# speechcatcher-asr/speechcatcher

Measured on AMD Instinct MI355X. Metric: concurrent real-time streams (audio-seconds/s), de_xl dims, 640 ms (10240-sample) chunk steps, beam 10 CTC+attention, higher is better.
Workload: dtype f32

## Files before the change

speechcatcher_amd/csrc/search.hip:

```cpp
#include "common.h"
#include "attn.h"
#include <mutex>
#include <unordered_map>

#define CTRL(s, f) sb.ctrl[(s) * 8 + (f)]
#define SC_CTC_T(s) (CTRL(s, SC_C_TCTC) > 0 ? CTRL(s, SC_C_TCTC) : CTRL(s, SC_C_T))

#define YSEQ(pp, s, h) (sb.yseq + (((long)(pp) * sb.S + (s)) * sb.W + (h)) * sb.LCAP)
#define XPOS(pp, s, h) (sb.xpos + (((long)(pp) * sb.S + (s)) * sb.W + (h)) * sb.LCAP)
#define ANC(pp, s) (sb.anc + ((long)(pp) * sb.S + (s)) * sb.LCAP * sb.W)
#define CTCR(pp, s) (sb.ctc_r + ((long)(pp) * sb.S + (s)) * sb.TCAP * 2 * sb.W)
#define CTCRS(pp, s) (sb.ctc_rs + ((long)(pp) * sb.S + (s)) * sb.TCAP * sb.W)

__global__ void ctc_extend_state_kernel(sc_search sb) {
  const int s = blockIdx.x, h = threadIdx.x;
  if (!CTRL(s, SC_C_ACTIVE) || !CTRL(s, SC_C_HAS)) return;
  const int T = CTRL(s, SC_C_T), told = CTRL(s, SC_C_TOLD), nh = CTRL(s, SC_C_NHYP);
  if (h >= nh || told >= T) return;
  float *r = CTCR(CTRL(s, SC_C_CUR), s);
  float *rs = CTCRS(CTRL(s, SC_C_CUR), s);
  const float *x = sb.ctcx + (long)s * sb.TCAP * sb.V;
  const int t0 = told < 1 ? 1 : told;
  float rb = r[((long)(t0 - 1) * 2 + 1) * sb.W + h];
  for (int t = t0; t < T; ++t) {
    rb = rb + x[(long)t * sb.V + sb.blank];
    r[((long)t * 2 + 0) * sb.W + h] = SC_LOGZERO;
    r[((long)t * 2 + 1) * sb.W + h] = rb;
    rs[(long)t * sb.W + h] = rb;
  }
}

__global__ __launch_bounds__(256) void ctc_table_transpose_kernel(sc_search sb) {
  __shared__ float tile[32][33];
  const int s = blockIdx.z;
  if (!CTRL(s, SC_C_ACTIVE)) return;
  const int T = CTRL(s, SC_C_T), told = CTRL(s, SC_C_TOLD);
  if (told >= T) return;
  const int V = sb.V, v0 = blockIdx.x * 32;
  const int tx = threadIdx.x & 31, ty = threadIdx.x >> 5;
  const float *x = sb.ctcx + (long)s * sb.TCAP * V;
  float *xt = sb.ctcxT + (long)s * V * sb.tct;
  for (int t0 = (told & ~31) + blockIdx.y * 32; t0 < T; t0 += gridDim.y * 32) {
#pragma unroll
    for (int j = 0; j < 4; ++j) {
      const int t = t0 + ty + 8 * j, v = v0 + tx;
      tile[ty + 8 * j][tx] = (t < T && v < V) ? x[(long)t * V + v] : 0.f;
    }
    __syncthreads();
#pragma unroll
    for (int j = 0; j < 4; ++j) {
      const int v = v0 + ty + 8 * j, t = t0 + tx;
      if (v < V && t >= told && t < T) xt[(long)v * sb.tct + t] = tile[tx][ty + 8 * j];
    }
    __syncthreads();
  }
}

extern "C" int sc_ctc_extend_state(const sc_search *sbp, void *stream) {
  SC_CHECK_ARG(sbp, "null");
  if (sbp->ctcxT)
    ctc_table_transpose_kernel<<<dim3(cdiv(sbp->V, 32), 4, sbp->S), 256, 0, (hipStream_t)stream>>>(*sbp);
  ctc_extend_state_kernel<<<sbp->S, 64, 0, (hipStream_t)stream>>>(*sbp);
  SC_CHECK_LAUNCH();
  return SC_OK;
}

__global__ void kv_rows_to_half_kernel(const float *stage, const int32_t *rows, int m, int TCAP, int d2, _Float16 *ckv) {
  const int li = blockIdx.y;
  for (long e = (long)blockIdx.x * blockDim.x + threadIdx.x; e < (long)m * d2; e += (long)gridDim.x * blockDim.x) {
    const int j = (int)(e / d2), c = (int)(e % d2);
    ckv[((long)rows[j] + (long)li * TCAP) * d2 + c] = (_Float16)stage[((long)li * m + j) * d2 + c];
  }
}

extern "C" int sc_kv_rows_to_half(const float *stage, const int32_t *rows, int m, int n_layers, int TCAP, int d2,
                                  void *ckv_half, void *stream) {
  SC_CHECK_ARG(stage && rows && ckv_half && m >= 0 && n_layers > 0 && d2 > 0, "bad arguments");
  if (m == 0) return SC_OK;
  const int gx = (int)(((long)m * d2 + 255) / 256 > 1024 ? 1024 : ((long)m * d2 + 255) / 256);
  kv_rows_to_half_kernel<<<dim3(gx, n_layers), 256, 0, (hipStream_t)stream>>>(stage, rows, m, TCAP, d2, (_Float16 *)ckv_half);
  SC_CHECK_LAUNCH();
  return SC_OK;
}

#define SC_KV_MAX_ROWS 65536
__global__ void dec_embed_kernel(sc_search sb, float sq) {
  const int row = blockIdx.x, s = row / sb.W, h = row % sb.W;
  if (!CTRL(s, SC_C_ACTIVE) || h >= CTRL(s, SC_C_NHYP)) return;
  const int L = CTRL(s, SC_C_L);
  const int tok = YSEQ(CTRL(s, SC_C_CUR), s, h)[L - 1];
  for (int c = threadIdx.x; c < sb.d; c += blockDim.x)
    sb.dx[(long)row * sb.d + c] = sb.embed[(long)tok * sb.d + c] * sq + sb.pe[(long)(L - 1) * sb.d + c];
}

extern "C" int sc_dec_embed(const sc_search *sbp, void *stream) {
  SC_CHECK_ARG(sbp, "null");
  dec_embed_kernel<<<sbp->S * sbp->W, 256, 0, (hipStream_t)stream>>>(*sbp, sqrtf((float)sbp->d));
  SC_CHECK_LAUNCH();
  return SC_OK;
}

template <int DK, int WM, bool SELF, int UNR, bool KVH = false>
__global__ __launch_bounds__(256, (UNR <= 4 && WM <= 10 && DK <= 32) ? 4 : 1) void dec_attn_flash_kernel(sc_search sb, int li) {
  constexpr int PCH = 128;
  constexpr int NTW = (UNR >= 8) ? 4 : 2;
  constexpr int NP = SELF ? 5 : 4;
  extern __shared__ __attribute__((aligned(16))) float smem[];
  const int head = blockIdx.x, s = sb.rowmap ? sb.rowmap[blockIdx.y * sb.W] / sb.W : blockIdx.y;
  if (!CTRL(s, SC_C_ACTIVE)) return;
  const int nh = CTRL(s, SC_C_NHYP);
  if (nh <= 0) return;
  const int L = CTRL(s, SC_C_L), cur = CTRL(s, SC_C_CUR), T = CTRL(s, SC_C_T);
  const int W = sb.W, d = sb.d;
  const int tid = threadIdx.x, lane = tid & 63, wave = tid >> 6;
  float *pm = smem;
  float *pl = pm + NP * 16;
  float *pO = pl + NP * 16;
  int *rows = (int *)(smem + mattn_partial_floats(DK, NP));
  int *wtot = rows + (SELF ? PCH * W : 0);
  float *qs = (float *)(wtot + 8);

  const float *qbase = SELF ? sb.dqkv + (long)s * W * 3 * d + head * DK : sb.dq + (long)s * W * d + head * DK;
  const int qld = SELF ? 3 * d : d;
  const long skv0 = ((long)s * sb.n_layers + li) * sb.kv_rows * 2 * d + head * DK;
  const long ckv0 = ((long)s * sb.n_layers + li) * sb.TCAP * 2 * d + head * DK;
  if (SELF) {
    const int *ancn = ANC(cur, s) + (long)(L - 1) * W;
    for (int e = tid; e < nh * DK; e += 256) {
      const int h = e / DK, c = e % DK;
      const long dst = skv0 + (long)ancn[h] * 2 * d;
      kv_store1<KVH>(sb.skv, dst + c, qbase[(long)h * 3 * d + d + c]);
      kv_store1<KVH>(sb.skv, dst + d + c, qbase[(long)h * 3 * d + 2 * d + c]);
    }
  }
  const float scale = sqrtf((float)DK);
  for (int e = tid; e < 16 * DK; e += 256) {
    const int h = e / DK, c = e % DK;
    qs[e] = h < nh ? qbase[(long)h * qld + c] / scale : 0.f;
  }
  MAttn<DK> st;
  mattn_init(st);

  if (SELF) {
    const int *anc = ANC(cur, s);
    const int Lc = L - 1;
    const int nchunk = cdiv(Lc, PCH);
    if (nchunk == 0) __syncthreads();
    int urows = nh;
    for (int ch = 0; ch < nchunk; ++ch) {
      const int c0 = ch * PCH;
      const int nopre[WM] = {};
      const int U = mattn_build_rows<WM>(rows, wtot, anc, c0, Lc, W, nh, tid, lane, wave, nopre);
      urows += U;
      mattn_walk<DK, NTW, KVH>(st, qs, sb.skv, d, cdiv(U, 16), wave, lane, [&](int idx, long &ke, unsigned &hm) {
        const int e = rows[min(idx, max(U - 1, 0))];
        hm = idx < U ? (unsigned)e >> 16 : 0u;
// ... 204 lines not shown

__device__ __forceinline__ int next_pow2(int v) {
  int n = 1;
  while (n < v) n <<= 1;
  return n;
}

__device__ __forceinline__ unsigned long long shfl_xor_u64(unsigned long long v, int mask) {
  const unsigned lo = __shfl_xor((unsigned)v, mask, 64), hi = __shfl_xor((unsigned)(v >> 32), mask, 64);
  return ((unsigned long long)hi << 32) | lo;
}
__device__ __forceinline__ unsigned long long shfl_u64(unsigned long long v, int src) {
  const unsigned lo = __shfl((unsigned)v, src, 64), hi = __shfl((unsigned)(v >> 32), src, 64);
  return ((unsigned long long)hi << 32) | lo;
}
__device__ __forceinline__ unsigned long long wave_sort64_desc(unsigned long long v, int lane) {
#pragma unroll
  for (int k = 2; k <= 64; k <<= 1) {
#pragma unroll
    for (int j = k >> 1; j > 0; j >>= 1) {
      const unsigned long long o = shfl_xor_u64(v, j);
      const bool keep_max = ((lane & j) == 0) == ((lane & k) == 0);
      v = keep_max ? (v > o ? v : o) : (v < o ? v : o);
    }
  }
  return v;
}
__device__ __forceinline__ unsigned long long wave_merge64_desc(unsigned long long a, unsigned long long b, int lane) {
  const unsigned long long br = shfl_u64(b, 63 - lane);
  unsigned long long v = a > br ? a : br;
#pragma unroll
  for (int j = 32; j > 0; j >>= 1) {
    const unsigned long long o = shfl_xor_u64(v, j);
    v = ((lane & j) == 0) ? (v > o ? v : o) : (v < o ? v : o);
  }
  return v;
}

__global__ __launch_bounds__(256) void logsoftmax_topk_kernel(sc_search sb) {
  __shared__ float red[8];
  __shared__ unsigned long long tops[4][64];
  const int row = blockIdx.x, s = row / sb.W, h = row % sb.W;
  if (!CTRL(s, SC_C_ACTIVE) || h >= CTRL(s, SC_C_NHYP)) return;
  const int V = sb.V, tid = threadIdx.x, lane = tid & 63, wave = tid >> 6;
  const float *x = sb.logits + (long)row * V;
  float xv[4];
  float m = -INFINITY;
#pragma unroll
  for (int q = 0; q < 4; ++q) {
    const int c = wave * 256 + q * 64 + lane;
    xv[q] = c < V ? x[c] : -INFINITY;
    m = fmaxf(m, xv[q]);
  }
  m = wave_max(m);
  if (lane == 0) red[wave] = m;
  __syncthreads();
  m = fmaxf(fmaxf(red[0], red[1]), fmaxf(red[2], red[3]));
  float sum = 0.f;
#pragma unroll
  for (int q = 0; q < 4; ++q) sum += (wave * 256 + q * 64 + lane < V) ? expf(xv[q] - m) : 0.f;
  sum = wave_sum(sum);
  if (lane == 0) red[4 + wave] = sum;
  __syncthreads();
  sum = (red[4] + red[5]) + (red[6] + red[7]);
  const float ls = logf(sum);
  unsigned long long key[4];
#pragma unroll
  for (int q = 0; q < 4; ++q) {
    const int c = wave * 256 + q * 64 + lane;
    if (c < V) {
      const float lp = (xv[q] - m) - ls;
      sb.logp[(long)row * V + c] = lp;
      key[q] = sort_key(__fmul_rn(sb.w_dec, lp), c);
    } else {
      key[q] = 0ull;
    }
  }
#pragma unroll
  for (int q = 0; q < 4; ++q) key[q] = wave_sort64_desc(key[q], lane);
  const unsigned long long m0 = wave_merge64_desc(key[0], key[1], lane);
  const unsigned long long m1 = wave_merge64_desc(key[2], key[3], lane);
  tops[wave][lane] = wave_merge64_desc(m0, m1, lane);
  __syncthreads();
  if (wave == 0) {
    const unsigned long long a = wave_merge64_desc(tops[0][lane], tops[1][lane], lane);
    const unsigned long long b = wave_merge64_desc(tops[2][lane], tops[3][lane], lane);
    const unsigned long long f = wave_merge64_desc(a, b, lane);
    if (lane < sb.K) sb.pre_ids[(long)row * sb.K + lane] = sort_key_index(f);
  }
}

__global__ __launch_bounds__(256) void logsoftmax_topk_sort_kernel(sc_search sb) {
  extern __shared__ __attribute__((aligned(16))) unsigned long long comp[];
  __shared__ float red[8];
  const int row = blockIdx.x, s = row / sb.W, h = row % sb.W;
  if (!CTRL(s, SC_C_ACTIVE) || h >= CTRL(s, SC_C_NHYP)) return;
  const int V = sb.V, tid = threadIdx.x, lane = tid & 63, wave = tid >> 6;
  const int NP = next_pow2(V);
  const float *x = sb.logits + (long)row * V;
  float m = -INFINITY;
  for (int c = tid; c < V; c += 256) m = fmaxf(m, x[c]);
  m = wave_max(m);
  if (lane == 0) red[wave] = m;
  __syncthreads();
  m = fmaxf(fmaxf(red[0], red[1]), fmaxf(red[2], red[3]));
  float sum = 0.f;
  for (int c = tid; c < V; c += 256) sum += expf(x[c] - m);
  sum = wave_sum(sum);
  if (lane == 0) red[4 + wave] = sum;
  __syncthreads();
  sum = (red[4] + red[5]) + (red[6] + red[7]);
  const float ls = logf(sum);
  for (int c = tid; c < NP; c += 256) {
    if (c < V) {
      float lp = (x[c] - m) - ls;
      sb.logp[(long)row * V + c] = lp;
      comp[c] = sort_key(__fmul_rn(sb.w_dec, lp), c);
    } else {
      comp[c] = 0ull;
    }
  }
  __syncthreads();
  block_bitonic_sort_desc(comp, NP);
  for (int k = tid; k < sb.K; k += 256) sb.pre_ids[(long)row * sb.K + k] = sort_key_index(comp[k]);
}

static size_t pow2_keys_bytes(int V) {
  size_t np = 1;
  while (np < (size_t)V) np <<= 1;
  return np * sizeof(unsigned long long);
}
static size_t fuse_topw_lds(int V) { return 2 * (size_t)V * sizeof(float) + pow2_keys_bytes(V); }

extern "C" int sc_logsoftmax_topk(const sc_search *sbp, void *stream) {
  SC_CHECK_ARG(sbp, "null");
  SC_CHECK_ARG(sbp->V > 0 && sbp->V <= SC_MAX_VOCAB, "vocabulary larger than SC_MAX_VOCAB (8192)");
  if (sbp->V <= 1024 && sbp->K <= 64)
    logsoftmax_topk_kernel<<<sbp->S * sbp->W, 256, 0, (hipStream_t)stream>>>(*sbp);
  else {
    const size_t lds = pow2_keys_bytes(sbp->V);
    const int rc = allow_large_lds(reinterpret_cast<const void *>(&logsoftmax_topk_sort_kernel), lds,
                                   pow2_keys_bytes(SC_MAX_VOCAB), "sc_logsoftmax_topk");
    if (rc != SC_OK) return rc;
    logsoftmax_topk_sort_kernel<<<sbp->S * sbp->W, 256, lds, (hipStream_t)stream>>>(*sbp);
  }
  SC_CHECK_LAUNCH();
  return SC_OK;
}

struct CtcChunkT {
  float4 xc[4], xb[4];
  float pn[16], pb[16];
};
#define SC_CTC_CK 16
__host__ __device__ static inline int ctc_tck(int TCAP) { return (TCAP + SC_CTC_CK - 1) / SC_CTC_CK; }
__device__ __forceinline__ void ctc_frame(float &r_n, float &r_b, float prs, float pb, bool same, float xc, float xb, float &phi) {
  phi = same ? pb : prs;
  const float nr_n = lse2(r_n, phi) + xc;
  const float nr_b = lse2(r_n, r_b) + xb;
  r_n = nr_n;
  r_b = nr_b;
}
__device__ __forceinline__ void ctc_psi_add(float &pm, float &ps, float v) {
  const float d = v - pm;
  const float e = sc_exp_neg(-fabsf(d));
  ps = d > 0.f ? ps * e + 1.f : ps + e;
  pm = sc_max_raw(pm, v);
}
__device__ __forceinline__ bool ctc_scan_is_split(int T, int L, int split_min) {
  const int out_len = L - 1;
  int start = out_len > 1 ? out_len : 1;
  if (start > T) start = T;
  return split_min > 0 && T - start >= split_min;
}
#define CTC_NSEG 32
static inline int ctc_split_min_ok(int TCAP, int split_min) { return ctc_tck(TCAP) >= CTC_NSEG ? split_min : 0; }

__global__ __launch_bounds__(256) void ctc_prefix_scan_colmajor_kernel(sc_search sb, int split_min) {
  const int s = blockIdx.y;
  if (!CTRL(s, SC_C_ACTIVE)) return;
  const int nh = CTRL(s, SC_C_NHYP), K = sb.K, W = sb.W, V = sb.V;
  const int e = blockIdx.x * 256 + threadIdx.x;
  if (e >= nh * K) return;
  const int h = e / K, k = e % K;
  const int T = SC_CTC_T(s), L = CTRL(s, SC_C_L), cur = CTRL(s, SC_C_CUR);
  if (ctc_scan_is_split(T, L, split_min)) return;
  const bool has = CTRL(s, SC_C_HAS);
  const long row = (long)s * W + h;
  const int c = sb.pre_ids[row * K + k];
  const int last = YSEQ(cur, s, h)[L - 1];
  const bool same = (c == last);
  const int tct = sb.tct;
  const float *__restrict__ xcol = sb.ctcxT + ((long)s * V + c) * tct;
  const float *__restrict__ xblk = sb.ctcxT + ((long)s * V + sb.blank) * tct;
  const float *__restrict__ rp = CTCR(cur, s);
  const float *__restrict__ rsp = CTCRS(cur, s);
  float *rn = sb.ctc_rnew + (long)s * ctc_tck(sb.TCAP) * 2 * (W * K);
  const int WK = W * K;
  const int out_len = L - 1;
  int start = out_len > 1 ? out_len : 1;
  if (start > T) start = T;
  for (int j = 0; SC_CTC_CK * j + SC_CTC_CK - 1 < start - 1; ++j) {
    rn[((long)j * 2) * WK + e] = SC_LOGZERO;
    rn[((long)j * 2 + 1) * WK + e] = SC_LOGZERO;
  }
  float r_n = (out_len == 0) ? xcol[0] : SC_LOGZERO;
  float r_b = SC_LOGZERO;
  if (((start - 1) & (SC_CTC_CK - 1)) == SC_CTC_CK - 1) {
    rn[((long)((start - 1) / SC_CTC_CK) * 2) * WK + e] = r_n;
    rn[((long)((start - 1) / SC_CTC_CK) * 2 + 1) * WK + e] = r_b;
  }
  float cum = 0.f;
  if (!has)
    for (int t = 0; t < start; ++t) cum += xblk[t];

  auto fetch = [&](CtcChunkT &q, int tb) {
#pragma unroll
    for (int j = 0; j < 4; ++j) {
      const int t4 = min(tb + 4 * j, tct - 4);
      q.xc[j] = *reinterpret_cast<const float4 *>(xcol + t4);
      q.xb[j] = *reinterpret_cast<const float4 *>(xblk + t4);
    }
    if (has) {
#pragma unroll
      for (int i = 0; i < 16; ++i) {
        int t = tb + i;
        t = t < T ? (t < 1 ? 1 : t) : T - 1;
        q.pn[i] = rsp[(long)(t - 1) * W + h];
        q.pb[i] = rp[((long)(t - 1) * 2 + 1) * W + h];
      }
    }
  };
  float pm = r_n, ps = 1.f;
  auto frame = [&](const CtcChunkT &q, int tb, int i) {
    const int t = tb + i;
    const float4 c4 = q.xc[i >> 2], b4 = q.xb[i >> 2];
    const float xc = (i & 3) == 0 ? c4.x : (i & 3) == 1 ? c4.y : (i & 3) == 2 ? c4.z : c4.w;
    const float xb = (i & 3) == 0 ? b4.x : (i & 3) == 1 ? b4.y : (i & 3) == 2 ? b4.z : b4.w;
    const float prs = has ? q.pn[i] : cum;
    const float pb = has ? q.pb[i] : cum;
    float phi;
    ctc_frame(r_n, r_b, prs, pb, same, xc, xb, phi);
    if ((i & (SC_CTC_CK - 1)) == SC_CTC_CK - 1) {
      rn[((long)(t / SC_CTC_CK) * 2) * WK + e] = r_n;
      rn[((long)(t / SC_CTC_CK) * 2 + 1) * WK + e] = r_b;
    }
    ctc_psi_add(pm, ps, phi + xc);
    if (!has) cum += xb;
  };
  auto advance = [&](const CtcChunkT &q, int tb) {
    if (tb >= start && tb + 16 <= T) {
#pragma unroll
      for (int i = 0; i < 16; ++i) frame(q, tb, i);
    } else {
#pragma unroll
      for (int i = 0; i < 16; ++i)
        if (tb + i >= start && tb + i < T) frame(q, tb, i);
    }
  };
  if (start < T) {
    CtcChunkT qa, qb;
    int tb = start & ~15;
    fetch(qa, tb);
    while (true) {
      if (tb + 16 < T) fetch(qb, tb + 16);
      advance(qa, tb);
      tb += 16;
      if (tb >= T) break;
      if (tb + 16 < T) fetch(qa, tb + 16);
      advance(qb, tb);
      tb += 16;
      if (tb >= T) break;
    }
  }
  float psi = pm + logf(ps);
  const float rsum_last = has ? rsp[(long)(T - 1) * W + h] : cum;
  if (c == sb.eos) psi = rsum_last;
  if (c == sb.blank) psi = SC_LOGZERO;
  sb.psi[row * K + k] = psi;
  if (k == 0) sb.psi_eos[row] = rsum_last;
}

#define CTC_EB (256 / CTC_NSEG)
__global__ __launch_bounds__(256) void ctc_prefix_scan_tpar_kernel(sc_search sb, int split_min) {
  __shared__ float co[8][CTC_NSEG][CTC_EB];
  __shared__ float st0[2][CTC_NSEG][CTC_EB];
  __shared__ float cum0[CTC_NSEG][CTC_EB];
  const int s = blockIdx.y;
  if (!CTRL(s, SC_C_ACTIVE)) return;
  const int nh = CTRL(s, SC_C_NHYP), K = sb.K, W = sb.W, V = sb.V;
  const int T = SC_CTC_T(s), L = CTRL(s, SC_C_L), cur = CTRL(s, SC_C_CUR);
  if (!ctc_scan_is_split(T, L, split_min)) return;
  if ((int)blockIdx.x * CTC_EB >= nh * K) return;
  const int el = threadIdx.x % CTC_EB, p = threadIdx.x / CTC_EB;
  const int e_raw = blockIdx.x * CTC_EB + el;
  const bool valid = e_raw < nh * K;
  const int e = valid ? e_raw : nh * K - 1;
  const int h = e / K, k = e % K;
  const bool has = CTRL(s, SC_C_HAS);
  const long row = (long)s * W + h;
  const int c = sb.pre_ids[row * K + k];
  const int last = YSEQ(cur, s, h)[L - 1];
  const bool same = (c == last);
  const int tct = sb.tct;
  const float *__restrict__ xcol = sb.ctcxT + ((long)s * V + c) * tct;
  const float *__restrict__ xblk = sb.ctcxT + ((long)s * V + sb.blank) * tct;
  const float *__restrict__ rp = CTCR(cur, s);
  const float *__restrict__ rsp = CTCRS(cur, s);
  float *rn = sb.ctc_rnew + (long)s * ctc_tck(sb.TCAP) * 2 * (W * K);
  const int WK = W * K;
  const int out_len = L - 1;
  int start = out_len > 1 ? out_len : 1;
  if (start > T) start = T;
  const float r_n0 = (out_len == 0) ? xcol[0] : SC_LOGZERO;
  const float r_b0 = SC_LOGZERO;
  const int base = start & ~15;
  const int seg = 16 * cdiv(T - base, 16 * CTC_NSEG);
  const int t_lo = max(start, base + p * seg), t_hi = min(T, base + (p + 1) * seg);

  auto fetch = [&](CtcChunkT &q, int tb) {
#pragma unroll
    for (int j = 0; j < 4; ++j) {
      const int t4 = min(tb + 4 * j, tct - 4);
      q.xc[j] = *reinterpret_cast<const float4 *>(xcol + t4);
      q.xb[j] = *reinterpret_cast<const float4 *>(xblk + t4);
    }
    if (has) {
#pragma unroll
      for (int i = 0; i < 16; ++i) {
        int t = tb + i;
        t = t < T ? (t < 1 ? 1 : t) : T - 1;
        q.pn[i] = rsp[(long)(t - 1) * W + h];
        q.pb[i] = rp[((long)(t - 1) * 2 + 1) * W + h];
      }
    }
  };
  auto walk = [&](int lo, int hi, auto body) {
    if (lo >= hi) return;
    CtcChunkT qa, qb;
    int tb = lo & ~15;
    fetch(qa, tb);
    while (true) {
      if (tb + 16 < hi) fetch(qb, tb + 16);
#pragma unroll
      for (int i = 0; i < 16; ++i)
        if (tb + i >= lo && tb + i < hi) body(qa, i, tb + i);
      tb += 16;
      if (tb >= hi) break;
      if (tb + 16 < hi) fetch(qa, tb + 16);
#pragma unroll
      for (int i = 0; i < 16; ++i)
        if (tb + i >= lo && tb + i < hi) body(qb, i, tb + i);
      tb += 16;
      if (tb >= hi) break;
    }
  };
  auto comp = [](const float4 &v, int i) { return (i & 3) == 0 ? v.x : (i & 3) == 1 ? v.y : (i & 3) == 2 ? v.z : v.w; };

  float cum = 0.f;
  if (!has) {
    float bs = 0.f;
    if (p == 0)
      for (int t = 0; t < start; ++t) bs += xblk[t];
    walk(t_lo, t_hi, [&](const CtcChunkT &q, int i, int) { bs += comp(q.xb[i >> 2], i); });
    co[7][p][el] = bs;
    __syncthreads();
    for (int q = 0; q < p; ++q) cum += co[7][q][el];
    if (p == 0) {
      cum = 0.f;
      for (int t = 0; t < start; ++t) cum += xblk[t];
    } else {
    }
    cum0[p][el] = cum;
  }
  float A = 0.f, C = SC_LOGZERO, D = 0.f, Un = SC_LOGZERO, Ub = SC_LOGZERO;
  float pm = SC_LOGZERO, ps = 0.f;
  {
    float cu = cum;
    walk(t_lo, t_hi, [&](const CtcChunkT &q, int i, int) {
      const float xc = comp(q.xc[i >> 2], i), xb = comp(q.xb[i >> 2], i);
      const float pb = has ? q.pb[i] : cu;
      const float phi = same ? pb : (has ? q.pn[i] : cu);
      const float nUb = lse2(Un, Ub) + xb;
      const float nC = lse2(A, C) + xb;
      Un = lse2(Un, phi) + xc;
      Ub = nUb;
      C = nC;
      A += xc;
      D += xb;
      ctc_psi_add(pm, ps, phi + xc);
      if (!has) cu += xb;
    });
  }
  co[0][p][el] = A; co[1][p][el] = C; co[2][p][el] = D; co[3][p][el] = Un; co[4][p][el] = Ub;
  co[5][p][el] = pm; co[6][p][el] = ps;
  __syncthreads();
  if (p == 0) {
    float n = r_n0, b = r_b0;
    float gm = r_n0, gs = 1.f;
    for (int q = 0; q < CTC_NSEG; ++q) {
      st0[0][q][el] = n;
      st0[1][q][el] = b;
      const float nn = lse2(co[0][q][el] + n, co[3][q][el]);
      const float nb = lse2(lse2(co[1][q][el] + n, co[2][q][el] + b), co[4][q][el]);
      n = nn;
      b = nb;
      const float m = sc_max_raw(gm, co[5][q][el]);
      gs = gs * sc_exp_neg(gm - m) + co[6][q][el] * sc_exp_neg(co[5][q][el] - m);
      gm = m;
    }
    if (valid) {
      float psi = gm + logf(gs);
      float total = 0.f;
      if (!has)
        for (int q = 0; q < CTC_NSEG; ++q) total += co[7][q][el];
      const float rsum_last = has ? rsp[(long)(T - 1) * W + h] : total;
      if (c == sb.eos) psi = rsum_last;
      if (c == sb.blank) psi = SC_LOGZERO;
      sb.psi[row * K + k] = psi;
      if (k == 0) sb.psi_eos[row] = rsum_last;
    }
  }
  __syncthreads();
  if (valid) {
    rn[((long)p * 2) * WK + e] = st0[0][p][el];
    rn[((long)p * 2 + 1) * WK + e] = st0[1][p][el];
  }
}

static std::mutex g_scan_split_mutex;
static std::unordered_map<const void *, int> g_scan_split;
static void scan_split_note(const sc_search *sbp, int eff) {
  std::lock_guard<std::mutex> lk(g_scan_split_mutex);
  g_scan_split[sbp->ctc_rnew] = eff;
}
static int scan_split_last(const sc_search *sbp) {
  std::lock_guard<std::mutex> lk(g_scan_split_mutex);
  auto it = g_scan_split.find(sbp->ctc_rnew);
  return it == g_scan_split.end() ? -1 : it->second;
}

extern "C" int sc_ctc_prefix_scan_split(const sc_search *sbp, int split_min, void *stream) {
  SC_CHECK_ARG(sbp, "null");
  SC_CHECK_ARG(sbp->ctcxT && sbp->tct >= 4 && sbp->tct % 4 == 0, "the prefix scan needs the column-major table copy (sc_search.ctcxT)");
  split_min = ctc_split_min_ok(sbp->TCAP, split_min);
  scan_split_note(sbp, split_min);
  dim3 grid(cdiv(sbp->W * sbp->K, 256), sbp->S);
  ctc_prefix_scan_colmajor_kernel<<<grid, 256, 0, (hipStream_t)stream>>>(*sbp, split_min);
  if (split_min > 0)
    ctc_prefix_scan_tpar_kernel<<<dim3(cdiv(sbp->W * sbp->K, CTC_EB), sbp->S), 256, 0, (hipStream_t)stream>>>(*sbp, split_min);
  SC_CHECK_LAUNCH();
  return SC_OK;
}

extern "C" int sc_ctc_prefix_scan(const sc_search *sbp, void *stream) { return sc_ctc_prefix_scan_split(sbp, 0, stream); }

__device__ __forceinline__ float sort_key_value(unsigned long long c) {
  unsigned u = (unsigned)(c >> 32);
  u = (u & 0x80000000u) ? (u & 0x7FFFFFFFu) : ~u;
  return __uint_as_float(u);
}

__global__ __launch_bounds__(256) void fuse_topw_kernel(sc_search sb) {
  extern __shared__ __attribute__((aligned(16))) float smem[];
  __shared__ int need_full;
  const int row = blockIdx.x, s = row / sb.W, h = row % sb.W;
  if (!CTRL(s, SC_C_ACTIVE) || h >= CTRL(s, SC_C_NHYP)) return;
  const int V = sb.V, K = sb.K, W = sb.W, tid = threadIdx.x;
  float *comb = smem, *ctc = smem + V;
  if (!(sb.w_ctc > 0.f)) {
    if (tid < W) {
      const int c = sb.pre_ids[(long)row * K + tid];
      sb.cand_tok[(long)row * W + tid] = c;
      sb.cand_score[(long)row * W + tid] = __fmul_rn(sb.w_dec, sb.logp[(long)row * V + c]);
      sb.cand_ctc[(long)row * W + tid] = 0.f;
    }
    return;
  }
  const float s_prev = CTRL(s, SC_C_HAS) ? sb.ctc_s[((long)CTRL(s, SC_C_CUR) * sb.S + s) * W + h] : 0.f;
  if (K < 64 && W <= 64 && sb.w_dec >= 0.f) {
    if (tid < 64) {
      const int lane = tid;
      int c = -1;
      float ps = SC_LOGZERO;
      if (lane < K) {
        c = sb.pre_ids[(long)row * K + lane];
        ps = sb.psi[(long)row * K + lane];
      }
      const bool eos_listed = __ballot(c == sb.eos) != 0ull;
      if (lane == K && !eos_listed) c = sb.eos;
      if (c == sb.eos) ps = sb.psi_eos[row];
      if (c == sb.blank) ps = SC_LOGZERO;
      unsigned long long key = 0ull;
      if (c >= 0) {
        const float cv = __fsub_rn(ps, s_prev);
        ctc[c] = cv;
        key = sort_key(__fadd_rn(__fmul_rn(sb.w_dec, sb.logp[(long)row * V + c]), __fmul_rn(sb.w_ctc, cv)), c);
      }
      key = wave_sort64_desc(key, lane);
      const float bound = __fmul_rn(sb.w_ctc, __fsub_rn(SC_LOGZERO, s_prev));
      const unsigned long long kw = shfl_u64(key, W - 1);
      const bool ok = kw != 0ull && sort_key_value(kw) > bound;
      if (lane == 0) need_full = ok ? 0 : 1;
      if (ok && lane < W) {
        const int i = sort_key_index(key);
        sb.cand_tok[(long)row * W + lane] = i;
        sb.cand_score[(long)row * W + lane] = sort_key_value(key);
        sb.cand_ctc[(long)row * W + lane] = ctc[i];
      }
    }
    __syncthreads();
    if (!need_full) return;
    __syncthreads();
  }
  for (int v = tid; v < V; v += 256) ctc[v] = SC_LOGZERO;
  __syncthreads();
  for (int k = tid; k < K; k += 256) ctc[sb.pre_ids[(long)row * K + k]] = sb.psi[(long)row * K + k];
  __syncthreads();
  if (tid == 0) {
    ctc[sb.eos] = sb.psi_eos[row];
    ctc[sb.blank] = SC_LOGZERO;
  }
  __syncthreads();
  for (int v = tid; v < V; v += 256) {
    const float cv = __fsub_rn(ctc[v], s_prev);
    ctc[v] = cv;
    comb[v] = __fadd_rn(__fmul_rn(sb.w_dec, sb.logp[(long)row * V + v]), __fmul_rn(sb.w_ctc, cv));
  }
  __syncthreads();
  const int NP = next_pow2(V);
  unsigned long long *comp = reinterpret_cast<unsigned long long *>(smem + 2 * V);
  for (int c = tid; c < NP; c += 256) comp[c] = c < V ? sort_key(comb[c], c) : 0ull;
  __syncthreads();
  block_bitonic_sort_desc(comp, NP);
  for (int k = tid; k < W; k += 256) {
    const int i = sort_key_index(comp[k]);
    sb.cand_tok[(long)row * W + k] = i;
    sb.cand_score[(long)row * W + k] = comb[i];
    sb.cand_ctc[(long)row * W + k] = ctc[i];
  }
}

extern "C" int sc_fuse_topw(const sc_search *sbp, void *stream) {
  SC_CHECK_ARG(sbp, "null");
  SC_CHECK_ARG(sbp->V > 0 && sbp->V <= SC_MAX_VOCAB, "vocabulary larger than SC_MAX_VOCAB (8192)");
  const size_t smem = fuse_topw_lds(sbp->V);
  const int rc = allow_large_lds(reinterpret_cast<const void *>(&fuse_topw_kernel), smem, fuse_topw_lds(SC_MAX_VOCAB),
                                 "sc_fuse_topw");
  if (rc != SC_OK) return rc;
  fuse_topw_kernel<<<sbp->S * sbp->W, 256, smem, (hipStream_t)stream>>>(*sbp);
  SC_CHECK_LAUNCH();
  return SC_OK;
}

__global__ __launch_bounds__(256) void beam_prune_kernel(sc_search sb) {
  extern __shared__ __attribute__((aligned(16))) double tot[];
  __shared__ int fl_any, fl_all, fl_best, fl_rep;
  __shared__ int win_h[64], win_tok[64];
  __shared__ unsigned bm[SC_KV_MAX_ROWS / 32];
  const int s = blockIdx.x, tid = threadIdx.x;
  if (!CTRL(s, SC_C_ACTIVE)) return;
  for (int w = tid; w < (sb.kv_rows + 31) / 32; w += 256) bm[w] = 0u;
  const int W = sb.W, K = sb.K;
  const int nh = CTRL(s, SC_C_NHYP), L = CTRL(s, SC_C_L), T = CTRL(s, SC_C_T);
  const int cur = CTRL(s, SC_C_CUR), o = 1 - cur;
  const int n = nh * W, nout = n < W ? n : W;
  if (tid == 0) { fl_any = 0; fl_all = 1; fl_best = 0; fl_rep = 0; }
  for (int e = tid; e < n; e += 256) {
    const int h = e / W, j = e % W;
    tot[e] = sb.score[((long)cur * sb.S + s) * W + h] + (double)sb.cand_score[((long)s * W + h) * W + j];
  }
  __syncthreads();
  for (int e = tid; e < n; e += 256) {
    const double te = tot[e];
    int rk = 0;
    for (int j = 0; j < n; ++j) rk += (tot[j] > te) || (tot[j] == te && j < e);
    if (rk >= nout) continue;
    const int h = e / W, j = e % W, i = rk;
    const long prow = (long)s * W + h;
    const int tok = sb.cand_tok[prow * W + j];
    win_h[i] = h;
    win_tok[i] = tok;
    const long oi = ((long)o * sb.S + s) * W + i, ci = ((long)cur * sb.S + s) * W + h;
    sb.score[oi] = te;
    sb.sc_dec[oi] = sb.sc_dec[ci] + (double)sb.logp[prow * sb.V + tok];
    sb.sc_ctc[oi] = sb.sc_ctc[ci] + (double)sb.cand_ctc[prow * W + j];
    int kk = -1;
    for (int q = 0; q < K; ++q)
      if (sb.pre_ids[prow * K + q] == tok) { kk = q; break; }
    float sval;
    if (tok == sb.blank) sval = SC_LOGZERO;
    else if (tok == sb.eos) sval = sb.psi_eos[prow];
    else if (kk >= 0) sval = sb.psi[prow * K + kk];
    else sval = SC_LOGZERO;
    sb.ctc_s[oi] = sval;
    sb.sel[((long)s * W + i) * 2] = h;
    sb.sel[((long)s * W + i) * 2 + 1] = kk < 0 ? 0 : kk;
    const bool is_eos = tok == sb.eos;
    if (is_eos) atomicOr(&fl_any, 1);
    else atomicAnd(&fl_all, 0);
    if (i == 0 && is_eos) atomicOr(&fl_best, 1);
  }
  __syncthreads();
  const int *asrc = ANC(cur, s);
  int *adst = ANC(o, s);
  bool rep = false;
  constexpr int UB = 4;
  const int ntot = nout * (L + 1);
  for (int e0 = tid; e0 < ntot; e0 += 256 * UB) {
    int yv[UB], xv[UB], av[UB];
#pragma unroll
    for (int u = 0; u < UB; ++u) {
      const int e = min(e0 + 256 * u, ntot - 1);
      const int i = e / (L + 1), p = min(e % (L + 1), L - 1);
      const int h = win_h[i];
      yv[u] = YSEQ(cur, s, h)[p];
      xv[u] = XPOS(cur, s, h)[p];
      av[u] = asrc[(long)p * W + h];
    }
#pragma unroll
    for (int u = 0; u < UB; ++u) {
      const int e = e0 + 256 * u;
      if (e >= ntot) break;
      const int i = e / (L + 1), p = e % (L + 1);
      const int tok = win_tok[i];
      int *ydst = YSEQ(o, s, i), *xdst = XPOS(o, s, i);
      if (p < L) {
        ydst[p] = yv[u];
        xdst[p] = xv[u];
        if (p >= 1 && yv[u] == tok && tok != sb.sos && tok != sb.eos) rep = true;
        adst[(long)p * W + i] = av[u];
        atomicOr(&bm[(av[u] >> 5) & (SC_KV_MAX_ROWS / 32 - 1)], 1u << (av[u] & 31));
      } else {
        ydst[L] = tok;
        xdst[L] = T - 1;
      }
    }
  }
  if (rep) atomicOr(&fl_rep, 1);
  __syncthreads();
  if (tid == 0)
    sb.flags[s] = (fl_any ? SC_F_ANY_EOS : 0) | (fl_best ? SC_F_BEST_EOS : 0) |
                  (fl_all ? SC_F_ALL_EOS : 0) | (fl_rep ? SC_F_REPEAT : 0);
  if (tid >= 64 || L + 1 > sb.LCAP) return;
  const int lane = tid, NR = sb.kv_rows, nwords = (NR + 31) / 32;
  int *out = adst + (long)L * W;
  int got = 0;
  for (int w0 = 0; w0 < nwords && got < nout; w0 += 64) {
    const int w = w0 + lane;
    unsigned fr = w < nwords ? ~bm[w] : 0u;
    if (w == nwords - 1 && (NR & 31)) fr &= (1u << (NR & 31)) - 1u;
    const int c = __popc(fr);
    int incl = c;
#pragma unroll
    for (int o2 = 1; o2 < 64; o2 <<= 1) {
      const int t = __shfl_up(incl, o2, 64);
      if (lane >= o2) incl += t;
    }
    int k = got + incl - c;
    while (fr && k < nout) {
      const int b = __ffs(fr) - 1;
      fr &= fr - 1u;
      out[k++] = w * 32 + b;
    }
    got += __shfl(incl, 63, 64);
  }
  if (got < nout && lane >= got && lane < nout) out[lane] = NR - 1;
  if (lane == 0 && sb.kvflags) sb.kvflags[s] = got < nout ? 1 : 0;
}

extern "C" int sc_beam_prune(const sc_search *sbp, void *stream) {
  SC_CHECK_ARG(sbp, "null");
  SC_CHECK_ARG(sbp->W <= 64, "beam wider than 64");
  SC_CHECK_ARG(sbp->kv_rows >= sbp->W && sbp->kv_rows <= SC_KV_MAX_ROWS, "kv_rows out of range (beam .. 65536)");
  size_t smem = (size_t)sbp->W * sbp->W * sizeof(double);
  beam_prune_kernel<<<sbp->S, 256, smem, (hipStream_t)stream>>>(*sbp);
  SC_CHECK_LAUNCH();
  return SC_OK;
}

__global__ __launch_bounds__(256) void ctc_gather_state_kernel(sc_search sb, int split_min) {
  const int s = blockIdx.y;
  if (!CTRL(s, SC_C_ACTIVE)) return;
  const int W = sb.W, K = sb.K, V = sb.V, T = SC_CTC_T(s), nh = CTRL(s, SC_C_NHYP), L = CTRL(s, SC_C_L);
  const int nout = nh * W < W ? nh * W : W;
  const int cur = CTRL(s, SC_C_CUR), o = 1 - cur;
  const bool has = CTRL(s, SC_C_HAS);
  const int WK = W * K, tct = sb.tct;
  float *dst = CTCR(o, s);
  float *dst_rs = CTCRS(o, s);
  const float *__restrict__ rp = CTCR(cur, s);
  const float *__restrict__ rsp = CTCRS(cur, s);
  const float *ck = sb.ctc_rnew + (long)s * ctc_tck(sb.TCAP) * 2 * WK;
  const int out_len = L - 1;
  int start = out_len > 1 ? out_len : 1;
  if (start > T) start = T;
  const bool split = ctc_scan_is_split(T, L, split_min);
  const int base = start & ~15;
  const int seg = split ? 16 * cdiv(T - base, 16 * CTC_NSEG) : SC_CTC_CK;
  const int nseg = split ? CTC_NSEG : cdiv(T, SC_CTC_CK);
  for (int idx = blockIdx.x * blockDim.x + threadIdx.x; idx < nout * nseg; idx += gridDim.x * blockDim.x) {
    const int i = idx % nout, j = idx / nout;
    const int h = sb.sel[((long)s * W + i) * 2], k = sb.sel[((long)s * W + i) * 2 + 1];
    const int e = h * K + k;
    const int c = sb.pre_ids[((long)s * W + h) * K + k];
    const bool same = c == YSEQ(cur, s, h)[L - 1];
    const float *__restrict__ xcol = sb.ctcxT + ((long)s * V + c) * tct;
    const float *__restrict__ xblk = sb.ctcxT + ((long)s * V + sb.blank) * tct;
    int t_lo, t_hi;
    float r_n, r_b;
    if (split) {
      t_lo = max(start, base + j * seg);
      t_hi = min(T, base + (j + 1) * seg);
      r_n = ck[((long)j * 2) * WK + e];
      r_b = ck[((long)j * 2 + 1) * WK + e];
      if (j == 0) {
        for (int t = 0; t < start - 1; ++t) {
          dst[((long)t * 2) * W + i] = SC_LOGZERO;
          dst[((long)t * 2 + 1) * W + i] = SC_LOGZERO;
          dst_rs[(long)t * W + i] = lse2(SC_LOGZERO, SC_LOGZERO);
        }
        dst[((long)(start - 1) * 2) * W + i] = (out_len == 0) ? xcol[0] : SC_LOGZERO;
        dst[((long)(start - 1) * 2 + 1) * W + i] = SC_LOGZERO;
        dst_rs[(long)(start - 1) * W + i] = lse2((out_len == 0) ? xcol[0] : SC_LOGZERO, SC_LOGZERO);
      }
    } else {
      const int t0 = j * SC_CTC_CK, t1 = min(t0 + SC_CTC_CK, T);
      if (t0 <= start - 1) {
        r_n = (out_len == 0) ? xcol[0] : SC_LOGZERO;
        r_b = SC_LOGZERO;
        for (int t = t0; t < min(start - 1, t1); ++t) {
          dst[((long)t * 2) * W + i] = SC_LOGZERO;
          dst[((long)t * 2 + 1) * W + i] = SC_LOGZERO;
          dst_rs[(long)t * W + i] = lse2(SC_LOGZERO, SC_LOGZERO);
        }
        if (start - 1 < t1) {
          dst[((long)(start - 1) * 2) * W + i] = r_n;
          dst[((long)(start - 1) * 2 + 1) * W + i] = r_b;
          dst_rs[(long)(start - 1) * W + i] = lse2(r_n, r_b);
        }
        t_lo = start;
      } else {
        r_n = ck[((long)(j - 1) * 2) * WK + e];
        r_b = ck[((long)(j - 1) * 2 + 1) * WK + e];
        t_lo = t0;
      }
      t_hi = t1;
    }
    if (t_lo >= t_hi) continue;
    float cum = 0.f;
    if (!has)
      for (int t = 0; t < t_lo; ++t) cum += xblk[t];
    for (int tb = t_lo & ~(SC_CTC_CK - 1); tb < t_hi; tb += SC_CTC_CK) {
      float xc[SC_CTC_CK], xb[SC_CTC_CK], pn[SC_CTC_CK], pb[SC_CTC_CK];
#pragma unroll
      for (int q = 0; q < SC_CTC_CK / 4; ++q) {
        const int t4 = min(tb + 4 * q, tct - 4);
        const float4 c4 = *reinterpret_cast<const float4 *>(xcol + t4), b4 = *reinterpret_cast<const float4 *>(xblk + t4);
        xc[4 * q] = c4.x; xc[4 * q + 1] = c4.y; xc[4 * q + 2] = c4.z; xc[4 * q + 3] = c4.w;
        xb[4 * q] = b4.x; xb[4 * q + 1] = b4.y; xb[4 * q + 2] = b4.z; xb[4 * q + 3] = b4.w;
      }
#pragma unroll
      for (int q = 0; q < SC_CTC_CK; ++q) {
        const int tp = min(max(tb + q - 1, 0), T - 1);
        pn[q] = has ? rsp[(long)tp * W + h] : 0.f;
        pb[q] = has ? rp[((long)tp * 2 + 1) * W + h] : 0.f;
      }
#pragma unroll
      for (int q = 0; q < SC_CTC_CK; ++q) {
        const int t = tb + q;
        if (t >= t_lo && t < t_hi) {
          float phi;
          ctc_frame(r_n, r_b, has ? pn[q] : cum, has ? pb[q] : cum, same, xc[q], xb[q], phi);
          dst[((long)t * 2) * W + i] = r_n;
          dst[((long)t * 2 + 1) * W + i] = r_b;
          dst_rs[(long)t * W + i] = lse2(r_n, r_b);
          if (!has) cum += xb[q];
        }
      }
    }
  }
}

extern "C" int sc_ctc_gather_state_split(const sc_search *sbp, int split_min, void *stream) {
  SC_CHECK_ARG(sbp, "null");
  SC_CHECK_ARG(sbp->ctcxT && sbp->tct >= 4, "the state rebuild needs the column-major table copy (sc_search.ctcxT)");
  int gx = cdiv(ctc_tck(sbp->TCAP) * sbp->W, 256);
  if (gx > 16) gx = 16;
  const int eff = ctc_split_min_ok(sbp->TCAP, split_min), last = scan_split_last(sbp);
  if (last >= 0 && last != eff) {
    sc_set_error("sc_ctc_gather_state_split: the last prefix scan of this batch ran with split_min = %d, the rebuild was asked for %d - "
                 "streams split over T leave segment states, not checkpoints: pass the scan's value (sc_ctc_gather_state() = 0)", last, eff);
    return SC_ERR_ARG;
  }
  ctc_gather_state_kernel<<<dim3(gx, sbp->S), 256, 0, (hipStream_t)stream>>>(*sbp, eff);
  SC_CHECK_LAUNCH();
  return SC_OK;
}

extern "C" int sc_ctc_gather_state(const sc_search *sbp, void *stream) { return sc_ctc_gather_state_split(sbp, 0, stream); }

static bool dec_fused_ok(const sc_search &sb) {
  if (const char *e = sc_hook("SC_DEC_FUSED"))
    return atoi(e) != 0 && sc_dec_layer_fused_supported(sb.d, sb.H, sb.W, sb.F) && sb.ph1 && sb.out_w_q;
  if (const char *e = sc_hook("SC_FUSED_MAX"))
    if ((sb.rowmap ? sb.n_rows : sb.S * sb.W) > atoi(e) && sc_dec_layer_hpw(sb) < 2) return false;
  return sc_dec_layer_fused_supported(sb.d, sb.H, sb.W, sb.F) && sb.ph1 && sb.ph2 && sb.ffn_part &&
         sb.max_ffn_part >= 1 && sb.out_w_q && sb.V % sb.d == 0 && sb.layers && sb.layers[0].wqkv_pp &&
         sb.layers[0].wq_pp && sb.layers[0].wo_pp && sb.layers[0].w1_p;
}

int sc_decode_step_form(const sc_search *sbp) { return dec_fused_ok(*sbp) ? (sc_dec_layer_stream_form(*sbp) ? 2 : 1) : 0; }

extern "C" int sc_decode_step(const sc_search *sbp, void *stream) { return sc_decode_step_ex(sbp, 0, stream); }

extern "C" int sc_decode_step_ex(const sc_search *sbp, int scan_split_min, void *stream) {
  SC_CHECK_ARG(sbp, "null");
  const sc_search &sb = *sbp;
  const int n = sb.rowmap ? sb.n_rows : sb.S * sb.W;
  int rc;
  if (dec_fused_ok(sb) && sc_dec_layer_stream_form(sb)) {
    float *xa = sb.dx, *xb = sb.dxn;
// ... 37 lines not shown
```

Baseline: 4089.

## Split CTC prefix scan into separate recurrence and psi threads per element

The column-major CTC prefix scan kernel now launches 512 threads per block. The lower 256 threads compute the r_n/r_b recurrence and checkpoint stores, while the upper 256 compute the psi log-sum-exp accumulation for the same elements. Each role skips the loads and arithmetic it does not need, and the phi source is now chosen by a pointer and stride once rather than loading both arrays. This shortens the serial dependency chain per thread, at the cost of redundant xcol/phi loads and higher register and occupancy pressure. Phase-timing stamp macros are also added, including under SC_PHASE_DBG.

New measurement: 4059. No clear change (-0.7%).

```diff
diff --git a/speechcatcher_amd/csrc/search.hip b/speechcatcher_amd/csrc/search.hip
--- a/speechcatcher_amd/csrc/search.hip
+++ b/speechcatcher_amd/csrc/search.hip
@@ -1,7 +1,31 @@
+#define SC_STAMP_ON (sc_tail_stamp_slot(sb))
 #include "common.h"
 #include "attn.h"
 #include <mutex>
 #include <unordered_map>
+
+__device__ __forceinline__ int sc_tail_stamp_slot(const sc_search &sb) {
+  const int rows = sb.rowmap ? sb.n_rows : sb.S * sb.W;
+  return rows >= 1000 ? 1 : rows <= 160 ? 2 : 0;
+}
+#ifdef SC_PHASE_DBG
+#define SC_TAIL_WAIT_DECL(acc) long long acc = 0
+#define SC_TAIL_WAIT(acc)                                       \
+  do {                                                          \
+    const long long w0__ = (long long)__builtin_amdgcn_s_memtime(); \
+    __builtin_amdgcn_s_waitcnt(0);                              \
+    acc += (long long)__builtin_amdgcn_s_memtime() - w0__;      \
+  } while (0)
+#define SC_TAIL_WAIT_PUT(k, i, cond, acc)                                                                         \
+  do {                                                                                                            \
+    const int wg__ = blockIdx.x + gridDim.x * blockIdx.y;                                                         \
+    if ((cond) && (SC_STAMP_ON) && wg__ < SC_PHASE_WGS) sc_phase_stamps[k][((SC_STAMP_ON) - 1) & (SC_PHASE_RING - 1)][wg__][i] = acc; \
+  } while (0)
+#else
+#define SC_TAIL_WAIT_DECL(acc) do {} while (0)
+#define SC_TAIL_WAIT(acc) do {} while (0)
+#define SC_TAIL_WAIT_PUT(k, i, cond, acc) do {} while (0)
+#endif
 
 #define CTRL(s, f) sb.ctrl[(s) * 8 + (f)]
 #define SC_CTC_T(s) (CTRL(s, SC_C_TCTC) > 0 ? CTRL(s, SC_C_TCTC) : CTRL(s, SC_C_T))
@@ -512,14 +536,21 @@
   float4 xc[4], xb[4];
   float pn[16], pb[16];
 };
+struct CtcScanChunk {
+  float4 xc[4], xb[4];
+  float phi[16];
+};
 #define SC_CTC_CK 16
 __host__ __device__ static inline int ctc_tck(int TCAP) { return (TCAP + SC_CTC_CK - 1) / SC_CTC_CK; }
-__device__ __forceinline__ void ctc_frame(float &r_n, float &r_b, float prs, float pb, bool same, float xc, float xb, float &phi) {
-  phi = same ? pb : prs;
+__device__ __forceinline__ void ctc_frame_phi(float &r_n, float &r_b, float phi, float xc, float xb) {
   const float nr_n = lse2(r_n, phi) + xc;
   const float nr_b = lse2(r_n, r_b) + xb;
   r_n = nr_n;
   r_b = nr_b;
+}
+__device__ __forceinline__ void ctc_frame(float &r_n, float &r_b, float prs, float pb, bool same, float xc, float xb, float &phi) {
+  phi = same ? pb : prs;
+  ctc_frame_phi(r_n, r_b, phi, xc, xb);
 }
 __device__ __forceinline__ void ctc_psi_add(float &pm, float &ps, float v) {
   const float d = v - pm;
@@ -536,16 +567,13 @@
 #define CTC_NSEG 32
 static inline int ctc_split_min_ok(int TCAP, int split_min) { return ctc_tck(TCAP) >= CTC_NSEG ? split_min : 0; }
 
-__global__ __launch_bounds__(256) void ctc_prefix_scan_colmajor_kernel(sc_search sb, int split_min) {
-  const int s = blockIdx.y;
-  if (!CTRL(s, SC_C_ACTIVE)) return;
-  const int nh = CTRL(s, SC_C_NHYP), K = sb.K, W = sb.W, V = sb.V;
-  const int e = blockIdx.x * 256 + threadIdx.x;
-  if (e >= nh * K) return;
+enum { SCAN_REC = 0, SCAN_PSI = 1 };
+template <bool HAS, int ROLE>
+__device__ __forceinline__ void ctc_scan_walk(const sc_search &sb, int s, int e, int T, int L, int cur) {
+  constexpr bool REC = ROLE == SCAN_REC, PSI = ROLE == SCAN_PSI;
+  [[maybe_unused]] constexpr int SR = ROLE == SCAN_PSI ? 1 : 0;
+  const int K = sb.K, W = sb.W, V = sb.V;
   const int h = e / K, k = e % K;
-  const int T = SC_CTC_T(s), L = CTRL(s, SC_C_L), cur = CTRL(s, SC_C_CUR);
-  if (ctc_scan_is_split(T, L, split_min)) return;
-  const bool has = CTRL(s, SC_C_HAS);
   const long row = (long)s * W + h;
   const int c = sb.pre_ids[row * K + k];
   const int last = YSEQ(cur, s, h)[L - 1];
@@ -553,62 +581,72 @@
   const int tct = sb.tct;
   const float *__restrict__ xcol = sb.ctcxT + ((long)s * V + c) * tct;
   const float *__restrict__ xblk = sb.ctcxT + ((long)s * V + sb.blank) * tct;
-  const float *__restrict__ rp = CTCR(cur, s);
   const float *__restrict__ rsp = CTCRS(cur, s);
+  const float *__restrict__ php = same ? CTCR(cur, s) + W + h : rsp + h;
+  const long pst = same ? 2 * W : W;
   float *rn = sb.ctc_rnew + (long)s * ctc_tck(sb.TCAP) * 2 * (W * K);
   const int WK = W * K;
   const int out_len = L - 1;
   int start = out_len > 1 ? out_len : 1;
   if (start > T) start = T;
-  for (int j = 0; SC_CTC_CK * j + SC_CTC_CK - 1 < start - 1; ++j) {
-    rn[((long)j * 2) * WK + e] = SC_LOGZERO;
-    rn[((long)j * 2 + 1) * WK + e] = SC_LOGZERO;
-  }
-  float r_n = (out_len == 0) ? xcol[0] : SC_LOGZERO;
-  float r_b = SC_LOGZERO;
-  if (((start - 1) & (SC_CTC_CK - 1)) == SC_CTC_CK - 1) {
-    rn[((long)((start - 1) / SC_CTC_CK) * 2) * WK + e] = r_n;
-    rn[((long)((start - 1) / SC_CTC_CK) * 2 + 1) * WK + e] = r_b;
-  }
-  float cum = 0.f;
-  if (!has)
-    for (int t = 0; t < start; ++t) cum += xblk[t];
-
-  auto fetch = [&](CtcChunkT &q, int tb) {
+
+  auto fetch = [&](CtcScanChunk &q, int tb) {
 #pragma unroll
     for (int j = 0; j < 4; ++j) {
       const int t4 = min(tb + 4 * j, tct - 4);
       q.xc[j] = *reinterpret_cast<const float4 *>(xcol + t4);
-      q.xb[j] = *reinterpret_cast<const float4 *>(xblk + t4);
-    }
-    if (has) {
+      if (REC || !HAS) q.xb[j] = *reinterpret_cast<const float4 *>(xblk + t4);
+    }
+    if (HAS) {
 #pragma unroll
       for (int i = 0; i < 16; ++i) {
         int t = tb + i;
         t = t < T ? (t < 1 ? 1 : t) : T - 1;
-        q.pn[i] = rsp[(long)(t - 1) * W + h];
-        q.pb[i] = rp[((long)(t - 1) * 2 + 1) * W + h];
+        q.phi[i] = php[(long)(t - 1) * pst];
       }
     }
   };
+  CtcScanChunk qa, qb;
+  int tb = start & ~15;
+  if (start < T) fetch(qa, tb);
+  if (REC)
+    for (int j = 0; SC_CTC_CK * j + SC_CTC_CK - 1 < start - 1; ++j) {
+      rn[((long)j * 2) * WK + e] = SC_LOGZERO;
+      rn[((long)j * 2 + 1) * WK + e] = SC_LOGZERO;
+    }
+  float r_n = (out_len == 0) ? xcol[0] : SC_LOGZERO;
+  float r_b = SC_LOGZERO;
+  if (REC && ((start - 1) & (SC_CTC_CK - 1)) == SC_CTC_CK - 1) {
+    rn[((long)((start - 1) / SC_CTC_CK) * 2) * WK + e] = r_n;
+    rn[((long)((start - 1) / SC_CTC_CK) * 2 + 1) * WK + e] = r_b;
+  }
+  float cum = 0.f;
+  if (!HAS)
+    for (int t = 0; t < start; ++t) cum += xblk[t];
+  SC_STAMP_BY(0, 1 + 4 * SR, (threadIdx.x & 255) == 0);
+
   float pm = r_n, ps = 1.f;
-  auto frame = [&](const CtcChunkT &q, int tb, int i) {
+  auto frame = [&](const CtcScanChunk &q, int tb, int i) {
     const int t = tb + i;
-    const float4 c4 = q.xc[i >> 2], b4 = q.xb[i >> 2];
+    const float4 c4 = q.xc[i >> 2];
     const float xc = (i & 3) == 0 ? c4.x : (i & 3) == 1 ? c4.y : (i & 3) == 2 ? c4.z : c4.w;
-    const float xb = (i & 3) == 0 ? b4.x : (i & 3) == 1 ? b4.y : (i & 3) == 2 ? b4.z : b4.w;
-    const float prs = has ? q.pn[i] : cum;
-    const float pb = has ? q.pb[i] : cum;
-    float phi;
-    ctc_frame(r_n, r_b, prs, pb, same, xc, xb, phi);
-    if ((i & (SC_CTC_CK - 1)) == SC_CTC_CK - 1) {
-      rn[((long)(t / SC_CTC_CK) * 2) * WK + e] = r_n;
-      rn[((long)(t / SC_CTC_CK) * 2 + 1) * WK + e] = r_b;
-    }
-    ctc_psi_add(pm, ps, phi + xc);
-    if (!has) cum += xb;
+    float xb = 0.f;
+    if (REC || !HAS) {
+      const float4 b4 = q.xb[i >> 2];
+      xb = (i & 3) == 0 ? b4.x : (i & 3) == 1 ? b4.y : (i & 3) == 2 ? b4.z : b4.w;
+    }
+    const float phi = HAS ? q.phi[i] : cum;
+    if (REC) {
+      ctc_frame_phi(r_n, r_b, phi, xc, xb);
+      if ((i & (SC_CTC_CK - 1)) == SC_CTC_CK - 1) {
+        rn[((long)(t / SC_CTC_CK) * 2) * WK + e] = r_n;
+        rn[((long)(t / SC_CTC_CK) * 2 + 1) * WK + e] = r_b;
+      }
+    }
+    if (PSI) ctc_psi_add(pm, ps, phi + xc);
+    if (!HAS) cum += xb;
   };
-  auto advance = [&](const CtcChunkT &q, int tb) {
+  auto advance = [&](const CtcScanChunk &q, int tb) {
     if (tb >= start && tb + 16 <= T) {
 #pragma unroll
       for (int i = 0; i < 16; ++i) frame(q, tb, i);
@@ -618,27 +656,50 @@
         if (tb + i >= start && tb + i < T) frame(q, tb, i);
     }
   };
+  SC_TAIL_WAIT_DECL(waited);
   if (start < T) {
-    CtcChunkT qa, qb;
-    int tb = start & ~15;
-    fetch(qa, tb);
     while (true) {
+      SC_TAIL_WAIT(waited);
       if (tb + 16 < T) fetch(qb, tb + 16);
       advance(qa, tb);
       tb += 16;
       if (tb >= T) break;
+      SC_TAIL_WAIT(waited);
       if (tb + 16 < T) fetch(qa, tb + 16);
       advance(qb, tb);
       tb += 16;
       if (tb >= T) break;
     }
   }
-  float psi = pm + logf(ps);
-  const float rsum_last = has ? rsp[(long)(T - 1) * W + h] : cum;
-  if (c == sb.eos) psi = rsum_last;
-  if (c == sb.blank) psi = SC_LOGZERO;
-  sb.psi[row * K + k] = psi;
-  if (k == 0) sb.psi_eos[row] = rsum_last;
+  SC_STAMP_BY(0, 2 + 4 * SR, (threadIdx.x & 255) == 0);
+  if (PSI) {
+    float psi = pm + logf(ps);
+    const float rsum_last = HAS ? rsp[(long)(T - 1) * W + h] : cum;
+    if (c == sb.eos) psi = rsum_last;
+    if (c == sb.blank) psi = SC_LOGZERO;
+    sb.psi[row * K + k] = psi;
+    if (k == 0) sb.psi_eos[row] = rsum_last;
+  }
+  SC_TAIL_WAIT_PUT(0, 4 + 4 * SR, (threadIdx.x & 255) == 0, waited);
+  SC_STAMP_BY(0, 3 + 4 * SR, (threadIdx.x & 255) == 0);
+}
+
+__global__ __launch_bounds__(512) void ctc_prefix_scan_colmajor_kernel(sc_search sb, int split_min) {
+  const int s = blockIdx.y;
+  if (!CTRL(s, SC_C_ACTIVE)) return;
+  SC_STAMP(0, 0);
+  const int e = blockIdx.x * 256 + (threadIdx.x & 255);
+  if (e >= CTRL(s, SC_C_NHYP) * sb.K) return;
+  const int T = SC_CTC_T(s), L = CTRL(s, SC_C_L), cur = CTRL(s, SC_C_CUR);
+  if (ctc_scan_is_split(T, L, split_min)) return;
+  const bool psi_lane = threadIdx.x >= 256;
+  if (CTRL(s, SC_C_HAS)) {
+    if (psi_lane) ctc_scan_walk<true, SCAN_PSI>(sb, s, e, T, L, cur);
+    else ctc_scan_walk<true, SCAN_REC>(sb, s, e, T, L, cur);
+  } else {
+    if (psi_lane) ctc_scan_walk<false, SCAN_PSI>(sb, s, e, T, L, cur);
+    else ctc_scan_walk<false, SCAN_REC>(sb, s, e, T, L, cur);
+  }
 }
 
 #define CTC_EB (256 / CTC_NSEG)
@@ -806,7 +867,7 @@
   split_min = ctc_split_min_ok(sbp->TCAP, split_min);
   scan_split_note(sbp, split_min);
   dim3 grid(cdiv(sbp->W * sbp->K, 256), sbp->S);
-  ctc_prefix_scan_colmajor_kernel<<<grid, 256, 0, (hipStream_t)stream>>>(*sbp, split_min);
+  ctc_prefix_scan_colmajor_kernel<<<grid, 512, 0, (hipStream_t)stream>>>(*sbp, split_min);
   if (split_min > 0)
     ctc_prefix_scan_tpar_kernel<<<dim3(cdiv(sbp->W * sbp->K, CTC_EB), sbp->S), 256, 0, (hipStream_t)stream>>>(*sbp, split_min);
   SC_CHECK_LAUNCH();
@@ -920,6 +981,7 @@
   __shared__ unsigned bm[SC_KV_MAX_ROWS / 32];
   const int s = blockIdx.x, tid = threadIdx.x;
   if (!CTRL(s, SC_C_ACTIVE)) return;
+  SC_STAMP(1, 0);
   for (int w = tid; w < (sb.kv_rows + 31) / 32; w += 256) bm[w] = 0u;
   const int W = sb.W, K = sb.K;
   const int nh = CTRL(s, SC_C_NHYP), L = CTRL(s, SC_C_L), T = CTRL(s, SC_C_T);
@@ -931,6 +993,7 @@
     tot[e] = sb.score[((long)cur * sb.S + s) * W + h] + (double)sb.cand_score[((long)s * W + h) * W + j];
   }
   __syncthreads();
+  SC_STAMP(1, 1);
   for (int e = tid; e < n; e += 256) {
     const double te = tot[e];
     int rk = 0;
@@ -962,6 +1025,7 @@
     if (i == 0 && is_eos) atomicOr(&fl_best, 1);
   }
   __syncthreads();
+  SC_STAMP(1, 2);
   const int *asrc = ANC(cur, s);
   int *adst = ANC(o, s);
   bool rep = false;
@@ -999,6 +1063,7 @@
   }
   if (rep) atomicOr(&fl_rep, 1);
   __syncthreads();
+  SC_STAMP(1, 3);
   if (tid == 0)
     sb.flags[s] = (fl_any ? SC_F_ANY_EOS : 0) | (fl_best ? SC_F_BEST_EOS : 0) |
                   (fl_all ? SC_F_ALL_EOS : 0) | (fl_rep ? SC_F_REPEAT : 0);
@@ -1027,7 +1092,9 @@
   }
   if (got < nout && lane >= got && lane < nout) out[lane] = NR - 1;
   if (lane == 0 && sb.kvflags) sb.kvflags[s] = got < nout ? 1 : 0;
-}
+  SC_STAMP_END(1, 4);
+}
+SC_PHASE_GETTER(sc_phase_debug_search)
 
 extern "C" int sc_beam_prune(const sc_search *sbp, void *stream) {
   SC_CHECK_ARG(sbp, "null");
```
